# PARC-projects/video-query-algorithms

Hardware: AMD Instinct MI355X
Metric: clips/sec TSN feature-extract (higher is better)
Workload: dtype f32; 1 GPU; configs[1]: TSN BN-Inception RGB, 224x224x3, T=3, B=32/GPU (96 crops/step), crops in HBM; global_batch=32, parallelism=dp1

## Files before the change

video-query-algorithms_amd/build.py:

```python
import os
import subprocess
import sys

HERE = os.path.dirname(os.path.abspath(__file__))
ROOT = os.path.dirname(HERE)
SOURCES = ["csrc/vq_sim.hip", "csrc/vq_tsn.hip", "csrc/vq_wino.hip", "csrc/vq_boot.hip", "csrc/vq_frames.hip", "csrc/vq_comm.hip", "csrc/vq_flow.hip",
           "csrc/vq_jpeg.hip", "csrc/vq_csv.hip", "csrc/vq_rounds.hip", "csrc/vq_round_targets.hip", "csrc/vq_round_topk.hip"]
HOST_SOURCES = ["csrc/host/vq_csv.cc", "csrc/host/vq_jpeg_host.cc", "csrc/host/vq_corners.cc", "csrc/host/vq_block_pool.cc", "csrc/host/vq_tsn_plan.cc", "csrc/host/vq_flow_host.cc", "csrc/host/vq_csv_read.cc"]
HEADERS = ["csrc/vq_common.h", "csrc/vq_tsn_kernels.h", "csrc/host/vq_host.h", "csrc/host/vq_jpeg_host.h", "csrc/host/vq_corners.h", "csrc/host/vq_block_pool.h", "csrc/host/vq_tsn_plan.h", "csrc/host/vq_flow_host.h", "../include/vq_amd.h", "../include/vq_amd_rows.h", "../include/vq_amd_csv.h", "../include/vq_amd_rounds.h", "../include/vq_amd_round_views.h", "../include/vq_amd_round_fit.h", "../include/vq_amd_round_targets.h", "../include/vq_amd_round_topk.h", "../include/vq_amd_round_grid.h", "../include/vq_amd_round_update.h", "../include/vq_amd_round_shard.h",
           "csrc/vq_db.h", "csrc/vq_tile_index.h", "csrc/vq_gauss_jordan.h", "csrc/vq_select.h", "csrc/vq_score.h", "csrc/vq_decimal.h", "csrc/vq_pow5_table.h", "csrc/host/vq_csv_read.h"]
OUT = os.path.join(HERE, "libvqamd.so")
FLAGS = ["-O3", "-std=c++17", "--offload-arch=gfx950", "-fPIC", "-ffp-contract=off", "-mllvm", "-amdgpu-mfma-vgpr-form=1", "-Wall", "-Wno-unused-result",
         "-I" + os.path.join(ROOT, "include"), "-I" + os.path.join(HERE, "csrc")]
FLAGS += os.environ.get("VQ_EXTRA_HIPCC_FLAGS", "").split()


def _stale():
    if not os.path.exists(OUT):
        return True
    t = os.path.getmtime(OUT)
    return any(os.path.getmtime(os.path.join(HERE, p)) > t for p in SOURCES + HOST_SOURCES + HEADERS + ["build.py"])


def build(force=False, verbose=True):
    if not force and not _stale():
        return OUT
    hipcc = os.environ.get("HIPCC", "/opt/rocm/bin/hipcc")
    objs = []
    procs = []
    os.makedirs(os.path.join(HERE, "build"), exist_ok=True)
    for src in SOURCES:
        obj = os.path.join(HERE, "build", os.path.basename(src) + ".o")
        objs.append(obj)
        cmd = [hipcc, "-c"] + FLAGS + [os.path.join(HERE, src), "-o", obj]
        if verbose:
            print(" ".join(cmd), flush=True)
        procs.append(subprocess.Popen(cmd))
    host_flags = ["-O3", "-std=c++17", "-fPIC", "-Wall", "-I" + os.path.join(ROOT, "include"), "-I" + os.path.join(HERE, "csrc"),
                  "-I" + os.path.join(HERE, "csrc", "host")]
    for src in HOST_SOURCES:
        obj = os.path.join(HERE, "build", os.path.basename(src) + ".o")
        objs.append(obj)
        cmd = [os.environ.get("CXX", "g++"), "-c"] + host_flags + [os.path.join(HERE, src), "-o", obj]
        if verbose:
            print(" ".join(cmd), flush=True)
        procs.append(subprocess.Popen(cmd))
    for p in procs:
        if p.wait() != 0:
            raise RuntimeError("compilation failed")
    cmd = [hipcc, "-shared", "--offload-arch=gfx950", "-fPIC"] + objs + ["-o", OUT]
    if verbose:
        print(" ".join(cmd), flush=True)
    subprocess.check_call(cmd + ["-ldl", "-lpthread"])
    return OUT


if __name__ == "__main__":
    build(force="--force" in sys.argv)
```

video-query-algorithms_amd/csrc/vq_tsn.hip:

```cpp
#include <algorithm>
#include <cmath>
#include <cstring>
#include <map>
#include <set>
#include <tuple>
#include <type_traits>
#include <vector>

#include "vq_common.h"
#include "vq_tsn_kernels.h"
#include "host/vq_block_pool.h"

using namespace vq;

typedef float floatx16 __attribute__((ext_vector_type(16)));
typedef float floatx4 __attribute__((ext_vector_type(4)));
typedef unsigned uintx4 __attribute__((__vector_size__(4 * sizeof(unsigned))));

__global__ void preprocess_kernel(const uint8_t* __restrict__ src, float* __restrict__ dst, int64_t nchunk, int C, int Cpad,
                                  const float* __restrict__ mean) {
    const int64_t i = (int64_t)blockIdx.x * blockDim.x + threadIdx.x;
    if (i >= nchunk) return;
    const int cpp = Cpad >> 2;
    const int64_t p = i / cpp;
// ... 684 lines not shown
    _Pragma("unroll") for (int i = 0; i < TM; ++i)                                                                  \
        fa[SET][i] = *reinterpret_cast<const floatx4*>(a_frag + 32 * i * pitch + (G) * 8);
#define VQ_PG_MFMA(SET, BSET, Q)                                                                                    \
    _Pragma("unroll") for (int s_ = 0; s_ < 4; ++s_)                                                                \
        _Pragma("unroll") for (int i = 0; i < TM; ++i)                                                              \
            _Pragma("unroll") for (int j = 0; j < TN; ++j)                                                          \
                acc[i][j] = __builtin_amdgcn_mfma_f32_32x32x2f32(fa[SET][i][s_], fbs[BSET][Q][j][s_], acc[i][j], 0, 0, 0);
#define VQ_PG_SLAB(S, BSET)                                                                                         \
    {                                                                                                               \
        const bool more = (S) + 1 < ns;                                                                             \
        if (more) {                                                                                                 \
            VQ_PG_FETCH_B((BSET) ^ 1, (S) + 1)                                                                      \
            VQ_PG_TAPS((S) + 1)                                              \
        }                                                                                                           \
        VQ_PG_FETCH_A(0, (S) * GS)                                                                                  \
        __builtin_amdgcn_sched_barrier(0);                                                                          \
        _Pragma("unroll") for (int q = 0; q < GS; ++q) {                                                            \
            if (q + 1 < GS) VQ_PG_FETCH_A((q + 1) & 1, (S) * GS + q + 1)                                            \
            __builtin_amdgcn_sched_barrier(0);                                                                      \
            VQ_PG_MFMA(q & 1, BSET, q)                                                                              \
            __builtin_amdgcn_sched_barrier(0);                                                                      \
        }                                                                                                           \
        if (more) {                                                                                                 \
            VQ_PG_POOL((S) + 1)                                                                                     \
            __syncthreads();                                  \
        }                                                                                                           \
    }

    const int ns = K / SLAB;
    VQ_PG_FETCH_B(0, 0)
    VQ_PG_TAPS(0)
    VQ_PG_POOL(0)
    __syncthreads();
    int s = 0;
    for (; s + 1 < ns; s += 2) {
        VQ_PG_SLAB(s, 0)
        VQ_PG_SLAB(s + 1, 1)
    }
    if (s < ns) VQ_PG_SLAB(s, 0)
#undef VQ_PG_SLAB
#undef VQ_PG_TAPS
#undef VQ_PG_POOL
#undef VQ_PG_FETCH_A
#undef VQ_PG_FETCH_B
#undef VQ_PG_MFMA
    VQ_EPILOGUE()
}

template <bool IS_MAX>
__global__ __launch_bounds__(256) void pool_kernel(PoolArgs a) {
    const int64_t i = (int64_t)blockIdx.x * blockDim.x + threadIdx.x;
    if (i < a.total) pool_one<IS_MAX>(a, i);
}

__global__ void gavgpool_kernel(const float* __restrict__ in, float* __restrict__ out, int n, int HW, int Cs_in, int coff_in,
                                int C, int Cs_out, int coff_out) {
    const int i = blockIdx.x * blockDim.x + threadIdx.x;
    if (i >= n * C) return;
    const int c = i % C, img = i / C;
    const float* p = in + (size_t)img * HW * Cs_in + coff_in + c;
    float acc = 0.f;
    for (int q = 0; q < HW; ++q) acc += p[(size_t)q * Cs_in];
    out[(size_t)img * Cs_out + coff_out + c] = acc / (float)HW;
}

constexpr int FC_ROWS = 4;
__global__ __launch_bounds__(64) void inner_product_kernel(const float* __restrict__ x, int x_stride, const float* __restrict__ W,
                                                           const float* __restrict__ bias, float* __restrict__ y, int y_stride, int M,
                                                           int K, int N) {
    const int lane = threadIdx.x;
    const int m0 = blockIdx.x * FC_ROWS, n0 = blockIdx.y * FC_COLS;
    const float* xr[FC_ROWS];
    const float* wr[FC_COLS];
#pragma unroll
    for (int r = 0; r < FC_ROWS; ++r) xr[r] = x + (size_t)min(m0 + r, M - 1) * x_stride;
#pragma unroll
    for (int c = 0; c < FC_COLS; ++c) wr[c] = W + (size_t)min(n0 + c, N - 1) * K;
    float acc[FC_ROWS][FC_COLS];
#pragma unroll
    for (int r = 0; r < FC_ROWS; ++r)
#pragma unroll
        for (int c = 0; c < FC_COLS; ++c) acc[r][c] = 0.f;
    for (int k = 4 * lane; k < K; k += 256) {
        floatx4 xv[FC_ROWS], wv[FC_COLS];
#pragma unroll
        for (int r = 0; r < FC_ROWS; ++r) xv[r] = *reinterpret_cast<const floatx4*>(xr[r] + k);
#pragma unroll
        for (int c = 0; c < FC_COLS; ++c) wv[c] = *reinterpret_cast<const floatx4*>(wr[c] + k);
#pragma unroll
        for (int e = 0; e < 4; ++e)
#pragma unroll
            for (int r = 0; r < FC_ROWS; ++r)
#pragma unroll
                for (int c = 0; c < FC_COLS; ++c) acc[r][c] = __builtin_fmaf(xv[r][e], wv[c][e], acc[r][c]);
    }
    float mine = 0.f;
#pragma unroll
    for (int r = 0; r < FC_ROWS; ++r)
#pragma unroll
        for (int c = 0; c < FC_COLS; ++c) {
            float v = acc[r][c];
#pragma unroll
            for (int s = 32; s >= 1; s >>= 1) v += __shfl_xor(v, s, 64);
            if (lane == r * FC_COLS + c) mine = v;
        }
    const int m = m0 + lane / FC_COLS, n = n0 + lane % FC_COLS;
    if (lane < FC_ROWS * FC_COLS && m < M && n < N) y[(size_t)m * y_stride + n] = mine + bias[n];
}

__global__ void splitk_combine_kernel(const float* __restrict__ part, int ksplit, size_t slice_stride, int M, int Cout,
                                      const float* __restrict__ bias, int relu, float* __restrict__ out, int Cs_out) {
    const int64_t i = (int64_t)blockIdx.x * blockDim.x + threadIdx.x;
    const int c4 = Cout / 4;
    if (i >= (int64_t)M * c4) return;
    const int m = (int)(i / c4), n = (int)(i - (int64_t)m * c4) * 4;
    floatx4 v = *reinterpret_cast<const floatx4*>(part + (size_t)m * Cout + n);
    for (int q = 1; q < ksplit; ++q) v += *reinterpret_cast<const floatx4*>(part + q * slice_stride + (size_t)m * Cout + n);
    v += *reinterpret_cast<const floatx4*>(bias + n);
    if (relu) {
        v[0] = fmaxf(v[0], 0.f);
        v[1] = fmaxf(v[1], 0.f);
        v[2] = fmaxf(v[2], 0.f);
        v[3] = fmaxf(v[3], 0.f);
    }
    *reinterpret_cast<floatx4*>(out + (size_t)m * Cs_out + n) = v;
}

__global__ void gavgpool_consensus_kernel(const float* __restrict__ in, float* __restrict__ out, double* __restrict__ feat, int T,
                                          int HW, int Cs_in, int coff_in, int C, int Cs_out, int coff_out) {
    __shared__ float pooled[kMaxFusedT][64];
    const int c = blockIdx.x * 64 + threadIdx.x, t = threadIdx.y, b = blockIdx.y;
    float v = 0.f;
    if (c < C) {
        const int img = b * T + t;
        const float* p = in + (size_t)img * HW * Cs_in + coff_in + c;
        float acc = 0.f;
        int q = 0;
        for (; q + 7 <= HW; q += 7) {
            float x[7];
#pragma unroll
            for (int u = 0; u < 7; ++u) x[u] = p[(size_t)(q + u) * Cs_in];
#pragma unroll
            for (int u = 0; u < 7; ++u) acc += x[u];
        }
        for (; q < HW; ++q) acc += p[(size_t)q * Cs_in];
        v = acc / (float)HW;
        out[(size_t)img * Cs_out + coff_out + c] = v;
    }
    pooled[t][threadIdx.x] = v;
    __syncthreads();
    if (t == 0 && c < C) {
        double cons = (double)pooled[0][threadIdx.x];
        for (int s = 1; s < T; ++s) cons = cons + (double)pooled[s][threadIdx.x];
        feat[(size_t)b * C + c] = cons / (double)T;
    }
}

__global__ void consensus_kernel(const float* __restrict__ per_snippet, double* __restrict__ feat, int B, int T, int D, int Cs) {
    const int i = blockIdx.x * blockDim.x + threadIdx.x;
    if (i >= B * D) return;
    const int d = i % D, b = i / D;
    double acc = (double)per_snippet[(size_t)(b * T) * Cs + d];
    for (int t = 1; t < T; ++t) acc = acc + (double)per_snippet[(size_t)(b * T + t) * Cs + d];
    feat[i] = acc / (double)T;
}

struct Launch {
    hipStream_t stream;
    hipEvent_t ev_start, ev_stop;
    int crop0;
    int T;
    bool fused_consensus;
};

struct vq_tsn {
    std::mutex mu;
    int device = 0;
    hipStream_t stream = nullptr;
// ... 242 lines not shown
    a.coff_out = L.dst_coff;
    a.Cout = L.cout;
    a.k = L.k;
    a.kw = L.k;
    a.col_off = 4;
    a.c_step = 0;
    a.stride = L.stride;
    a.pad = L.pad;
    a.M = n_crops * td.h * td.w;
    a.Kp = (L.k * L.k * L.cin + KPAD - 1) / KPAD * KPAD;
    a.relu = L.relu;
    a.pool_k = L.pre_pool_k;
    a.pool_s = L.pre_pool_stride;
    a.ksplit = 1;
    a.k_per = 0;
    a.seg_stride = 0;
    a.tiles_m = a.tiles_n = 0;
    a.in_bytes = (unsigned)((size_t)n_crops * ts.h * ts.w * ts.c * sizeof(float));
    a.w_bytes = (unsigned)((size_t)L.cout * a.Kp * sizeof(float));
}

static int launch_conv_layer(const vq_tsn* net, const Launch& ln, int li, int n_crops, int tile_idx) {
    ConvArgs a;
    fill_conv_args(net, ln, li, n_crops, a);
    const vq_layer_desc& L = net->plan.layers[li];
    const bool stem_rows = L.src == 0 && net->plan.input.s2d_pad >= 0 && net->plan.input.s2d_order == 1;
    if (stem_rows) {
        a.k = a.kw = 1;
        a.Cin = 4 * L.k * L.cin;
        a.col_off = net->plan.tensors[L.src].w * net->plan.tensors[L.src].c;
        a.c_step = 4;
        a.Kp = stem_rows_kp(net->plan.input.c);
        a.w_bytes = (unsigned)((size_t)L.cout * a.Kp * sizeof(float));
    } else if (L.pad == 0 && L.k > 1 && L.cin == net->plan.tensors[L.src].c && L.src_coff == 0) {
        a.kw = 1;
        a.Cin = L.k * L.cin;
    }
    const ConvLaunch run = conv_launch(net, li, a, stem_rows, tile_idx);
    const ConvTile& t = kTiles[tile_idx];
    if (!run) return fail(VQ_E_INVALID, "layer %d: no kernel for tile %dx%dx%d pipe=%d", li, t.bm, t.bn, t.bk, t.pipe);
    if (net->plan.ksplit[li] == 1) return run(ln, a);
    a.ksplit = net->plan.ksplit[li];
    a.k_per = a.Kp / a.ksplit;
    a.seg_stride = (L.cout + 31) / 32;
    a.bias = net->zero_bias;
    a.out_row0 = (int)cdiv((int64_t)ln.crop0 * (int64_t)net->plan.split_crop_floats, (int64_t)L.cout);
    Launch slices = ln, combine = ln;
    slices.ev_stop = nullptr;
    combine.ev_start = nullptr;
    const int rc = run(slices, a);
    if (rc != VQ_OK) return rc;
    const vq_tensor_desc& td = net->plan.tensors[L.dst];
    float* out = net->slots[L.dst] + (size_t)ln.crop0 * td.h * td.w * td.c + L.dst_coff;
    const int64_t work = (int64_t)a.M * (L.cout / 4);
    VQ_LAUNCH(splitk_combine_kernel, (unsigned)cdiv(work, 256), 256, 0, combine.stream, combine.ev_start, combine.ev_stop,
              net->split_scratch + (size_t)a.out_row0 * L.cout, a.ksplit, net->split_slice_floats, a.M, L.cout, net->blob + L.b_off, L.relu, out, td.c);
    VQ_CHECK_LAUNCH();
    return VQ_OK;
}

static void fill_wino_job(const vq_tsn* net, const Launch& ln, int li, int n_crops, WinoJob& a, int variant) {
    const vq_layer_desc& L = net->plan.layers[li];
    const vq_tensor_desc& ts = net->plan.tensors[L.src];
    const vq_tensor_desc& td = net->plan.tensors[L.dst];
    memset(&a, 0, sizeof a);
    a.in = net->slots[L.src] + (size_t)ln.crop0 * ts.h * ts.w * ts.c;
    a.u = net->blob + L.w_off;
    a.bias = net->blob + L.b_off;
    a.out = net->slots[L.dst] + (size_t)ln.crop0 * td.h * td.w * td.c;
    a.H = ts.h;
    a.W = ts.w;
    a.Cs_in = ts.c;
    a.coff_in = L.src_coff;
    a.Cin = L.cin;
    a.Cs_out = td.c;
    a.coff_out = L.dst_coff;
    a.Cout = L.cout;
    a.th = (ts.h + 1) / 2;
    a.tw = (ts.w + 1) / 2;
    a.P = n_crops * a.th * a.tw;
    a.relu = L.relu;
    a.t16 = L.op == VQ_OP_CONV_WINOGRAD16 && variant >= 2;
    if (a.t16) a.u += (size_t)16 * L.cout * L.cin;
    a.in_bytes = (unsigned)((size_t)n_crops * ts.h * ts.w * ts.c * sizeof(float));
    a.out_bytes = (unsigned)((size_t)n_crops * td.h * td.w * td.c * sizeof(float));
    a.u_bytes = (unsigned)((size_t)16 * L.cout * L.cin * sizeof(float));
}

static void fill_pool_args(const vq_tsn* net, const Launch& ln, int li, int n_crops, PoolArgs& a) {
    const vq_layer_desc& L = net->plan.layers[li];
    const vq_tensor_desc& ts = net->plan.tensors[L.src];
    const vq_tensor_desc& td = net->plan.tensors[L.dst];
    memset(&a, 0, sizeof a);
    a.in = net->slots[L.src] + (size_t)ln.crop0 * ts.h * ts.w * ts.c;
    a.out = net->slots[L.dst] + (size_t)ln.crop0 * td.h * td.w * td.c;
    a.H = ts.h;
    a.W = ts.w;
    a.Cs_in = ts.c;
    a.coff_in = L.src_coff;
    a.C = L.cin;
    a.Ho = td.h;
    a.Wo = td.w;
    a.Cs_out = td.c;
    a.coff_out = L.dst_coff;
    a.k = L.k;
    a.stride = L.stride;
    a.pad = L.pad;
    a.is_max = L.op == VQ_OP_MAXPOOL;
    a.total = (int64_t)n_crops * td.h * td.w * (L.cin / 4);
    a.bias = (L.op == VQ_OP_AVGPOOL && L.has_bias) ? net->blob + L.b_off : nullptr;
    a.relu = (L.op == VQ_OP_AVGPOOL) ? L.relu : 0;
}

static int launch_wino_layers(const vq_tsn* net, const Launch& ln, const std::vector<int>& members, int n_crops, int variant) {
    WinoGroup g;
    memset(&g, 0, sizeof g);
    for (int li : members) {
        if (is_wino(net->plan.layers[li].op)) {
            VQ_REQUIRE(g.n_jobs < kWinoMaxJobs, "a Winograd launch carries at most %d convolutions", kWinoMaxJobs);
            fill_wino_job(net, ln, li, n_crops, g.job[g.n_jobs++], variant);
        } else {
            VQ_REQUIRE(g.n_pools < kWinoMaxPools, "a Winograd launch carries at most %d pooling layers", kWinoMaxPools);
            fill_pool_args(net, ln, li, n_crops, g.pool[g.n_pools++]);
        }
    }
    bool both = true;
    for (int li : members)
        if (net->plan.layers[li].op == VQ_OP_CONV_WINOGRAD) both = false;
    if (variant >= 2 && !both) {
        variant -= 2;
        for (int q = 0; q < g.n_jobs; ++q) VQ_REQUIRE(!g.job[q].t16, "internal: mixed Winograd layouts in one launch");
    }
    return launch_wino_group(g, variant, ln.stream, ln.ev_start, ln.ev_stop);
}

static int run_layer(const vq_tsn* net, const Launch& ln, int li, int n_crops, int tune_key);

static int run_item(const vq_tsn* net, const Launch& whole, const LaunchItem& it, int n_crops, int tune_key) {
    for (int done = 0; done < n_crops;) {
        const int n = std::min(n_crops - done, it.max_crops);
        Launch ln = whole;
        ln.crop0 = whole.crop0 + done;
        if (done != 0) ln.ev_start = nullptr;
        if (done + n != n_crops) ln.ev_stop = nullptr;
        int rc;
        if (it.kind == 1) {
            auto tn = net->tuned.find(tune_key);
            rc = launch_wino_layers(net, ln, it.layers, n, tn != net->tuned.end() ? tn->second[it.layers[0]] : 0);
        } else {
            rc = run_layer(net, ln, it.layers[0], n, tune_key);
        }
        if (rc != VQ_OK) return rc;
        done += n;
    }
    return VQ_OK;
}

constexpr int kPairedKey = 1 << 24;
static inline int tile_key(int n_crops, bool paired) { return n_crops + (paired ? kPairedKey : 0); }

struct EventSet {
    std::vector<hipEvent_t> ev;
    ~EventSet() {
        for (hipEvent_t e : ev)
// ... 74 lines not shown
        int win = seen.empty() ? 0 : seen[0].second;
        for (size_t k = 0; k < std::min<size_t>(3, seen.size()) && seen.size() > 1; ++k) {
            for (int m : it.layers) pick[m] = seen[k].second;
            float ms = 0.f;
            const int rc = timed(it, 5, &ms);
            if (rc != VQ_OK) return rc;
            if (ms < best) {
                best = ms;
                win = seen[k].second;
            }
        }
        for (int m : it.layers) pick[m] = win;
    }
    return VQ_OK;
}

static int ensure_tuned(vq_tsn* net, int n_crops, bool paired) {
    const int key = tile_key(n_crops, paired);
    if (net->forced_tile >= 0 || net->tuned.find(key) != net->tuned.end()) return VQ_OK;
    for (const bool p : {paired, !paired}) {
        std::vector<int> sizes;
        for (const auto& kv : net->tuned)
            if ((kv.first >= kPairedKey) == p && !net->tuned_borrowed.count(kv.first)) sizes.push_back(kv.first - (p ? kPairedKey : 0));
        if (const int nearest = nearest_size(sizes, n_crops)) {
            net->tuned[key] = net->tuned[tile_key(nearest, p)];
            net->tuned_borrowed.insert(key);
            return VQ_OK;
        }
    }
    if (!net->autotune) return VQ_OK;
    return autotune(net, n_crops, paired);
}

static int run_layer(const vq_tsn* net, const Launch& ln, int li, int n_crops, int tune_key) {
    const vq_layer_desc& L = net->plan.layers[li];
    const vq_tensor_desc& ts = net->plan.tensors[L.src];
    const vq_tensor_desc& td = net->plan.tensors[L.dst];
    if (L.op == VQ_OP_CONV) {
        int t = net->forced_tile;
        if (t < 0) {
            auto it = net->tuned.find(tune_key);
            t = it != net->tuned.end() ? it->second[li] : heuristic_tile(net, li, n_crops);
        }
        return launch_conv_layer(net, ln, li, n_crops, t);
    }
    if (is_wino(L.op)) {
        auto it = net->tuned.find(tune_key);
        return launch_wino_layers(net, ln, std::vector<int>{li}, n_crops, it != net->tuned.end() ? it->second[li] : 0);
    }
    if (L.op == VQ_OP_MAXPOOL || L.op == VQ_OP_AVGPOOL) {
        PoolArgs a;
        fill_pool_args(net, ln, li, n_crops, a);
        const int64_t blocks = (a.total + 255) / 256;
        if (L.op == VQ_OP_MAXPOOL)
            VQ_LAUNCH(pool_kernel<true>, (unsigned)blocks, 256, 0, ln.stream, ln.ev_start, ln.ev_stop, a);
        else
            VQ_LAUNCH(pool_kernel<false>, (unsigned)blocks, 256, 0, ln.stream, ln.ev_start, ln.ev_stop, a);
        VQ_CHECK_LAUNCH();
        return VQ_OK;
    }
    if (L.op == VQ_OP_GLOBAL_AVGPOOL) {
        const float* gin = net->slots[L.src] + (size_t)ln.crop0 * ts.h * ts.w * ts.c;
        float* gout = net->slots[L.dst] + (size_t)ln.crop0 * td.c;
        const int T = ln.T;
        if (li == net->plan.consensus_layer && ln.fused_consensus) {
            const int B = n_crops / T;
            VQ_LAUNCH(gavgpool_consensus_kernel, dim3(cdiv(L.cin, 64), B), dim3(64, T), 0, ln.stream, ln.ev_start, ln.ev_stop, gin, gout,
                      net->feat_dev + (size_t)(ln.crop0 / T) * net->plan.D, T, ts.h * ts.w, ts.c, L.src_coff, L.cin, td.c, L.dst_coff);
        } else {
            VQ_LAUNCH(gavgpool_kernel, cdiv((int64_t)n_crops * L.cin, 256), 256, 0, ln.stream, ln.ev_start, ln.ev_stop, gin, gout, n_crops,
                      ts.h * ts.w, ts.c, L.src_coff, L.cin, td.c, L.dst_coff);
        }
        VQ_CHECK_LAUNCH();
        return VQ_OK;
    }
    if (L.op == VQ_OP_INNER_PRODUCT) {
        const float* xin = net->slots[L.src] + (size_t)ln.crop0 * ts.c + L.src_coff;
        float* yout = net->slots[L.dst] + (size_t)ln.crop0 * td.c + L.dst_coff;
        VQ_LAUNCH(inner_product_kernel, dim3(cdiv(n_crops, FC_ROWS), cdiv(L.cout, FC_COLS)), 64, 0, ln.stream, ln.ev_start, ln.ev_stop, xin, ts.c,
                  net->blob + L.w_off, net->blob + L.b_off, yout, td.c, n_crops, L.cin, L.cout);
        VQ_CHECK_LAUNCH();
        return VQ_OK;
    }
    return fail(VQ_E_INVALID, "layer %d: unknown op %d", li, L.op);
}

extern "C" {

int vq_tsn_create(const vq_tensor_desc* tensors, int32_t n_tensors, const vq_layer_desc* layers, int32_t n_layers,
                  const vq_conv_segment* segments, int32_t n_segments, const float* blob_host, int64_t blob_floats,
                  const vq_input_desc* input, int32_t feature_slot, int32_t max_crops, int32_t device, vq_tsn** out) {
    VQ_REQUIRE(out, "out is NULL");
    *out = nullptr;
    TsnPlan plan;
    const int vrc = validate_plan(tensors, n_tensors, layers, n_layers, segments, n_segments, blob_host, blob_floats, input, feature_slot, max_crops, &plan);
    if (vrc != VQ_OK) return vrc;
    const int in_channels = input->c;
    int ndev = 0;
    VQ_HIP(hipGetDeviceCount(&ndev));
    VQ_REQUIRE(device >= 0 && device < ndev, "device %d out of range (%d visible)", device, ndev);
    DeviceGuard g(device);
    auto* net = new vq_tsn;
    net->device = device;
    net->max_crops = max_crops;
    net->in_channels = in_channels;
    net->plan = std::move(plan);
    net->feature_slot = feature_slot;
// ... 499 lines not shown
```

video-query-algorithms_amd/csrc/vq_tsn_kernels.h:

```cpp
#pragma once
#include <hip/hip_runtime.h>
#include <hip/hip_ext.h>

#include "host/vq_tsn_plan.h"

namespace vq {

__device__ __forceinline__ int xcd_remap(int bid, int nwg) {
    const int q = nwg >> 3, r = nwg & 7, xcd = bid & 7, idx = bid >> 3;
    return (xcd < r ? xcd * (q + 1) : r * (q + 1) + (xcd - r) * q) + idx;
}

__device__ __forceinline__ unsigned magic_div(unsigned x, unsigned m) { return m ? __umulhi(x, m) : x; }

struct FullDiv {
    unsigned m, sh1, sh2;
};
__device__ __forceinline__ unsigned full_div(unsigned x, const FullDiv& d) {
    const unsigned t = __umulhi(d.m, x);
    return (t + ((x - t) >> d.sh1)) >> d.sh2;
}
static inline FullDiv full_div_for(unsigned d) {
    unsigned l = 0;
    while ((1ull << l) < d) ++l;
    FullDiv f;
    f.m = (unsigned)(((1ull << 32) * ((1ull << l) - d)) / d + 1);
    f.sh1 = l < 1 ? l : 1;
    f.sh2 = l > 1 ? l - 1 : 0;
    return f;
}
constexpr int kRecipShift = 22;
__device__ __forceinline__ unsigned umul24(unsigned x, unsigned y_uniform) {
    unsigned r;
    asm("v_mul_u32_u24 %0, %2, %1" : "=v"(r) : "v"(x), "s"(y_uniform));
    return r;
}
__device__ __forceinline__ int imul24(int x, int y_uniform) {
    int r;
    asm("v_mul_i32_i24 %0, %2, %1" : "=v"(r) : "v"(x), "s"(y_uniform));
    return r;
}
static inline unsigned recip22(unsigned d) { return (1u << kRecipShift) / d + 1u; }
static inline bool recip22_ok(unsigned d, unsigned xmax) {
    return d >= 1 && (unsigned long long)xmax * d < (1ull << kRecipShift) && (unsigned long long)xmax * recip22(d) < (1ull << 32);
}

struct PoolArgs {
    const float* in;
    float* out;
    int H, W, Cs_in, coff_in, C;
    int Ho, Wo, Cs_out, coff_out;
    int k, stride, pad;
    int is_max;
    int64_t total;
    const float* bias;
    int relu;
    int unit0, n_units;
};
constexpr int kPoolPerWG = 1024;

template <bool IS_MAX>
__device__ __forceinline__ void pool_one(const PoolArgs& a, int64_t i) {
    const int c4n = a.C >> 2;
    const int c4 = (int)(i % c4n);
    int64_t pix = i / c4n;
    const int pw = (int)(pix % a.Wo);
    pix /= a.Wo;
    const int ph = (int)(pix % a.Ho);
    const int64_t n = pix / a.Ho;
    int hs = ph * a.stride - a.pad, ws = pw * a.stride - a.pad;
    int he = min(hs + a.k, a.H + a.pad), we = min(ws + a.k, a.W + a.pad);
    const float pool_size = (float)((he - hs) * (we - ws));
    hs = max(hs, 0);
    ws = max(ws, 0);
    he = min(he, a.H);
    we = min(we, a.W);
    const float* base = a.in + (size_t)n * a.H * a.W * a.Cs_in + a.coff_in + c4 * 4;
    float4 acc = IS_MAX ? make_float4(-INFINITY, -INFINITY, -INFINITY, -INFINITY) : make_float4(0.f, 0.f, 0.f, 0.f);
    for (int h = hs; h < he; ++h)
        for (int w = ws; w < we; ++w) {
            const float4 v = *reinterpret_cast<const float4*>(base + ((size_t)h * a.W + w) * a.Cs_in);
            if (IS_MAX) {
                acc.x = fmaxf(acc.x, v.x);
                acc.y = fmaxf(acc.y, v.y);
                acc.z = fmaxf(acc.z, v.z);
                acc.w = fmaxf(acc.w, v.w);
            } else {
                acc.x += v.x;
                acc.y += v.y;
                acc.z += v.z;
                acc.w += v.w;
            }
        }
    if (!IS_MAX) {
        acc.x /= pool_size;
        acc.y /= pool_size;
        acc.z /= pool_size;
        acc.w /= pool_size;
        if (a.bias) {
            const float4 b = *reinterpret_cast<const float4*>(a.bias + c4 * 4);
            acc.x += b.x;
            acc.y += b.y;
            acc.z += b.z;
            acc.w += b.w;
        }
        if (a.relu) {
            acc.x = fmaxf(acc.x, 0.f);
            acc.y = fmaxf(acc.y, 0.f);
            acc.z = fmaxf(acc.z, 0.f);
            acc.w = fmaxf(acc.w, 0.f);
        }
    }
// ... 47 lines not shown
```

video-query-algorithms_amd/csrc/vq_wino.hip:

```cpp
#include "vq_common.h"
#include "vq_tsn_kernels.h"

using namespace vq;

typedef float floatx16 __attribute__((ext_vector_type(16)));
typedef float floatx4 __attribute__((ext_vector_type(4)));
typedef float floatx2 __attribute__((ext_vector_type(2)));
typedef unsigned uintx4 __attribute__((__vector_size__(4 * sizeof(unsigned))));

namespace {

__device__ __forceinline__ floatx2 pk_add2(floatx2 x, floatx2 y) {
    floatx2 r;
    asm("v_pk_add_f32 %0, %1, %2" : "=v"(r) : "v"(x), "v"(y));
    return r;
}
__device__ __forceinline__ floatx2 pk_sub2(floatx2 x, floatx2 y) {
    floatx2 r;
    asm("v_pk_add_f32 %0, %1, %2 neg_lo:[0,1] neg_hi:[0,1]" : "=v"(r) : "v"(x), "v"(y));
    return r;
}
__device__ __forceinline__ floatx4 pk_add(floatx4 x, floatx4 y) {
    const floatx2 lo = pk_add2(x.xy, y.xy), hi = pk_add2(x.zw, y.zw);
    return (floatx4){lo.x, lo.y, hi.x, hi.y};
// ... 391 lines not shown
    for (int nb = 0; nb < NB; ++nb) {
#pragma unroll
        for (int bb = 0; bb < 2; ++bb) {
            const int b = 2 * nb + bb;
            floatx4 t0, t1;
#pragma unroll
            for (int h2 = 0; h2 < 2; ++h2) {
                const floatx2 m0 = {acc[0][b][2 * h2], acc[0][b][2 * h2 + 1]}, m1 = {acc[1][b][2 * h2], acc[1][b][2 * h2 + 1]};
                const floatx2 m2 = {acc[2][b][2 * h2], acc[2][b][2 * h2 + 1]}, m3 = {acc[3][b][2 * h2], acc[3][b][2 * h2 + 1]};
                const floatx2 s0 = pk_add2(pk_add2(m0, m1), m2), s1 = pk_sub2(pk_sub2(m1, m2), m3);
                t0[2 * h2] = s0.x;
                t0[2 * h2 + 1] = s0.y;
                t1[2 * h2] = s1.x;
                t1[2 * h2 + 1] = s1.y;
            }
            *reinterpret_cast<floatx4*>(ep_w + 16 * bb) = t0;
            *reinterpret_cast<floatx4*>(ep_w + BP16 * EP_ROW + 16 * bb) = t1;
        }
        __syncthreads();
        {
            const floatx4 v0 = *reinterpret_cast<const floatx4*>(ep_r + (0 * 2 + bsel) * BP16 * EP_ROW);
            const floatx4 v1 = *reinterpret_cast<const floatx4*>(ep_r + (1 * 2 + bsel) * BP16 * EP_ROW);
            const floatx4 v2 = *reinterpret_cast<const floatx4*>(ep_r + (2 * 2 + bsel) * BP16 * EP_ROW);
            const floatx4 v3 = *reinterpret_cast<const floatx4*>(ep_r + (3 * 2 + bsel) * BP16 * EP_ROW);
            floatx4 y0 = pk_add(pk_add(v0, v1), v2);
            floatx4 y1 = pk_sub(pk_sub(v1, v2), v3);
            if (a.relu) {
#pragma unroll
                for (int r = 0; r < 4; ++r) {
                    y0[r] = relu1(y0[r]);
                    y1[r] = relu1(y1[r]);
                }
            }
            const bool blk_ok = n0 + 32 * nb < a.Cout;
            __builtin_amdgcn_raw_buffer_store_b128(__builtin_bit_cast(uintx4, y0), out_rsrc, blk_ok ? ooff[0] : 0xFFFFFFFFu, nb * (32 * 4), 0);
            __builtin_amdgcn_raw_buffer_store_b128(__builtin_bit_cast(uintx4, y1), out_rsrc, blk_ok ? ooff[1] : 0xFFFFFFFFu, nb * (32 * 4), 0);
        }
        if (nb + 1 < NB) __syncthreads();
    }
}

template <int NB, int TB>
__global__ __launch_bounds__(256) __attribute__((amdgpu_waves_per_eu(NB == 1 ? 4 : 2, NB == 1 ? 4 : 2)))
void wino_f2x2_3x3_kernel(WinoGroup g) {
    extern __shared__ __attribute__((aligned(16))) char smem_raw[];
    float* hs = reinterpret_cast<float*>(smem_raw);
    const int b = blockIdx.x;
    if (b >= g.pool_unit0) {
        int q = 0;
        if (g.n_pools > 1 && b >= g.pool[1].unit0) q = 1;
        const PoolArgs& pa = g.pool[q];
        const int unit = b - pa.unit0;
        if (unit >= pa.n_units) return;
#pragma unroll
        for (int r = 0; r < kPoolPerWG / 256; ++r) {
            const int64_t i = (int64_t)unit * kPoolPerWG + r * 256 + threadIdx.x;
            if (i < pa.total) {
                if (pa.is_max)
                    pool_one<true>(pa, i);
                else
                    pool_one<false>(pa, i);
            }
        }
        return;
    }
    int j = 0;
#pragma unroll
    for (int q = 1; q < kWinoMaxJobs; ++q)
        if (q < g.n_jobs && b >= g.job[q].unit0) j = q;
    const WinoJob& a = g.job[j];
    const int unit = b - a.unit0;
    if (unit >= a.n_units) return;
    if constexpr (TB == 16)
        wino16_unit<NB>(a, unit, hs);
    else
        wino_unit<NB>(a, unit, hs);
}

unsigned magic_u32(unsigned d) { return d == 1 ? 0u : (unsigned)(0x100000000ull / d) + 1u; }

template <int NB, int TB>
int launch_t(WinoGroup& g, hipStream_t stream, hipEvent_t ev_start, hipEvent_t ev_stop) {
    int units = 0;
    for (int q = 0; q < g.n_jobs; ++q) {
        WinoJob& a = g.job[q];
        a.tiles_n = cdiv(a.Cout, 32 * NB);
        const long long n = (long long)cdiv(a.P, TB) * a.tiles_n;
        VQ_REQUIRE(n > 0 && n < (1 << 24), "Winograd job %d: %lld workgroups", q, n);
        a.unit0 = units;
        a.n_units = (int)n;
        units += ((int)n + 7) & ~7;
        const unsigned tpi = (unsigned)(a.th * a.tw);
        VQ_REQUIRE((unsigned long long)n * a.tiles_n < 0x100000000ull && (unsigned long long)(a.P + BP) * tpi < 0x100000000ull &&
                       recip22_ok((unsigned)a.tw, (unsigned)a.tw + BP) && recip22_ok((unsigned)a.th, (unsigned)a.th + BP + 2),
                   "Winograd job %d: shape outside the reciprocal-division range", q);
        VQ_REQUIRE((unsigned long long)cdiv(a.P, (int)tpi) * a.H * a.W < (1ull << 23) && a.Cs_in < (1 << 23) && a.Cs_out < (1 << 23),
                   "Winograd job %d: more than 2^23 pixels in a slot (split the batch)", q);
        a.m_tiles_n = magic_u32((unsigned)a.tiles_n);
        a.m_tpi = magic_u32(tpi);
        a.m_tw = magic_u32((unsigned)a.tw);
        a.s_tw = recip22((unsigned)a.tw);
        a.s_th = recip22((unsigned)a.th);
    }
    g.pool_unit0 = units;
    for (int q = 0; q < g.n_pools; ++q) {
        PoolArgs& pa = g.pool[q];
// ... 38 lines not shown
```

Before: 12580 clips/s.

## Add specialized 3x3 pooling path with buffer loads and 2D split-K combine grid

Adds a fast pooling path for 3x3 stride-1 pad-1 and stride-2 pad-0 pools. It uses reciprocal-based 24-bit index math, raw buffer loads with out-of-range masking for padding, packed adds, max3, and software-pipelined tap fetches. The path is used both as a standalone kernel and inside the fused Winograd group. The split-K combine kernel is also reshaped to a 2D grid with 32-bit offsets, guarded by a new size check. Both changes aim to cut integer division cost and 64-bit addressing overhead in memory-bound stages, at the cost of more code and tight range preconditions.

```diff
diff --git a/video-query-algorithms_amd/build.py b/video-query-algorithms_amd/build.py
--- a/video-query-algorithms_amd/build.py
+++ b/video-query-algorithms_amd/build.py
@@ -7,7 +7,7 @@
 SOURCES = ["csrc/vq_sim.hip", "csrc/vq_tsn.hip", "csrc/vq_wino.hip", "csrc/vq_boot.hip", "csrc/vq_frames.hip", "csrc/vq_comm.hip", "csrc/vq_flow.hip",
            "csrc/vq_jpeg.hip", "csrc/vq_csv.hip", "csrc/vq_rounds.hip", "csrc/vq_round_targets.hip", "csrc/vq_round_topk.hip"]
 HOST_SOURCES = ["csrc/host/vq_csv.cc", "csrc/host/vq_jpeg_host.cc", "csrc/host/vq_corners.cc", "csrc/host/vq_block_pool.cc", "csrc/host/vq_tsn_plan.cc", "csrc/host/vq_flow_host.cc", "csrc/host/vq_csv_read.cc"]
-HEADERS = ["csrc/vq_common.h", "csrc/vq_tsn_kernels.h", "csrc/host/vq_host.h", "csrc/host/vq_jpeg_host.h", "csrc/host/vq_corners.h", "csrc/host/vq_block_pool.h", "csrc/host/vq_tsn_plan.h", "csrc/host/vq_flow_host.h", "../include/vq_amd.h", "../include/vq_amd_rows.h", "../include/vq_amd_csv.h", "../include/vq_amd_rounds.h", "../include/vq_amd_round_views.h", "../include/vq_amd_round_fit.h", "../include/vq_amd_round_targets.h", "../include/vq_amd_round_topk.h", "../include/vq_amd_round_grid.h", "../include/vq_amd_round_update.h", "../include/vq_amd_round_shard.h",
+HEADERS = ["csrc/vq_common.h", "csrc/vq_tsn_kernels.h", "csrc/vq_div9.h","csrc/host/vq_host.h", "csrc/host/vq_jpeg_host.h", "csrc/host/vq_corners.h", "csrc/host/vq_block_pool.h", "csrc/host/vq_tsn_plan.h", "csrc/host/vq_flow_host.h", "../include/vq_amd.h", "../include/vq_amd_rows.h", "../include/vq_amd_csv.h", "../include/vq_amd_rounds.h", "../include/vq_amd_round_views.h", "../include/vq_amd_round_fit.h", "../include/vq_amd_round_targets.h", "../include/vq_amd_round_topk.h", "../include/vq_amd_round_grid.h", "../include/vq_amd_round_update.h", "../include/vq_amd_round_shard.h",
            "csrc/vq_db.h", "csrc/vq_tile_index.h", "csrc/vq_gauss_jordan.h", "csrc/vq_select.h", "csrc/vq_score.h", "csrc/vq_decimal.h", "csrc/vq_pow5_table.h", "csrc/host/vq_csv_read.h"]
 OUT = os.path.join(HERE, "libvqamd.so")
 FLAGS = ["-O3", "-std=c++17", "--offload-arch=gfx950", "-fPIC", "-ffp-contract=off", "-mllvm", "-amdgpu-mfma-vgpr-form=1", "-Wall", "-Wno-unused-result",
diff --git a/video-query-algorithms_amd/csrc/vq_div9.h b/video-query-algorithms_amd/csrc/vq_div9.h
--- /dev/null
+++ b/video-query-algorithms_amd/csrc/vq_div9.h
@@ -0,0 +1,19 @@
+#pragma once
+
+#if defined(__HIPCC__)
+#define VQ_DIV9_FN __host__ __device__ __forceinline__
+#else
+#define VQ_DIV9_FN static inline
+#endif
+
+namespace vq {
+
+VQ_DIV9_FN float div9(float a) {
+    const float z = 1.0f / 9.0f;
+    const float q = a * z;
+    const float r = __builtin_fmaf(-9.0f, q, a);
+    const float c = __builtin_fmaf(r, z, q);
+    return (q == 0.0f || __builtin_isinf(q)) ? q : c;
+}
+
+}
diff --git a/video-query-algorithms_amd/csrc/vq_tsn.hip b/video-query-algorithms_amd/csrc/vq_tsn.hip
--- a/video-query-algorithms_amd/csrc/vq_tsn.hip
+++ b/video-query-algorithms_amd/csrc/vq_tsn.hip
@@ -760,6 +760,7 @@
     const int64_t i = (int64_t)blockIdx.x * blockDim.x + threadIdx.x;
     if (i < a.total) pool_one<IS_MAX>(a, i);
 }
+__global__ __launch_bounds__(256) void pool_fast_kernel(PoolArgs a) { pool_unit_any(a, blockIdx.x); }
 
 __global__ void gavgpool_kernel(const float* __restrict__ in, float* __restrict__ out, int n, int HW, int Cs_in, int coff_in,
                                 int C, int Cs_out, int coff_out) {
@@ -816,14 +817,16 @@
     if (lane < FC_ROWS * FC_COLS && m < M && n < N) y[(size_t)m * y_stride + n] = mine + bias[n];
 }
 
-__global__ void splitk_combine_kernel(const float* __restrict__ part, int ksplit, size_t slice_stride, int M, int Cout,
-                                      const float* __restrict__ bias, int relu, float* __restrict__ out, int Cs_out) {
-    const int64_t i = (int64_t)blockIdx.x * blockDim.x + threadIdx.x;
-    const int c4 = Cout / 4;
-    if (i >= (int64_t)M * c4) return;
-    const int m = (int)(i / c4), n = (int)(i - (int64_t)m * c4) * 4;
-    floatx4 v = *reinterpret_cast<const floatx4*>(part + (size_t)m * Cout + n);
-    for (int q = 1; q < ksplit; ++q) v += *reinterpret_cast<const floatx4*>(part + q * slice_stride + (size_t)m * Cout + n);
+__global__ __launch_bounds__(256) void splitk_combine_kernel(const float* __restrict__ part, int ksplit, size_t slice_stride, int M, int Cout,
+                                                             const float* __restrict__ bias, int relu, float* __restrict__ out, int Cs_out) {
+    const unsigned m = blockIdx.x * 4u + (threadIdx.x >> 6), n = (blockIdx.y * 64u + (threadIdx.x & 63u)) * 4u;
+    if (m >= (unsigned)M || n >= (unsigned)Cout) return;
+    const unsigned at = m * (unsigned)Cout + n;
+    floatx4 v = *reinterpret_cast<const floatx4*>(part + at);
+    for (int q = 1; q < ksplit; ++q) {
+        part += slice_stride;
+        v += *reinterpret_cast<const floatx4*>(part + at);
+    }
     v += *reinterpret_cast<const floatx4*>(bias + n);
     if (relu) {
         v[0] = fmaxf(v[0], 0.f);
@@ -831,7 +834,7 @@
         v[2] = fmaxf(v[2], 0.f);
         v[3] = fmaxf(v[3], 0.f);
     }
-    *reinterpret_cast<floatx4*>(out + (size_t)m * Cs_out + n) = v;
+    *reinterpret_cast<floatx4*>(out + (m * (unsigned)Cs_out + n)) = v;
 }
 
 __global__ void gavgpool_consensus_kernel(const float* __restrict__ in, float* __restrict__ out, double* __restrict__ feat, int T,
@@ -1180,8 +1183,8 @@
     if (rc != VQ_OK) return rc;
     const vq_tensor_desc& td = net->plan.tensors[L.dst];
     float* out = net->slots[L.dst] + (size_t)ln.crop0 * td.h * td.w * td.c + L.dst_coff;
-    const int64_t work = (int64_t)a.M * (L.cout / 4);
-    VQ_LAUNCH(splitk_combine_kernel, (unsigned)cdiv(work, 256), 256, 0, combine.stream, combine.ev_start, combine.ev_stop,
+    VQ_REQUIRE((int64_t)a.M * L.cout < (1ll << 31) && (int64_t)a.M * td.c < (1ll << 31), "layer %d: K-split combine pass beyond 32-bit offsets (split the batch)", li);
+    VQ_LAUNCH(splitk_combine_kernel, dim3((unsigned)cdiv(a.M, 4), (unsigned)cdiv(L.cout / 4, 64)), 256, 0, combine.stream, combine.ev_start, combine.ev_stop,
               net->split_scratch + (size_t)a.out_row0 * L.cout, a.ksplit, net->split_slice_floats, a.M, L.cout, net->blob + L.b_off, L.relu, out, td.c);
     VQ_CHECK_LAUNCH();
     return VQ_OK;
@@ -1238,6 +1241,10 @@
     a.total = (int64_t)n_crops * td.h * td.w * (L.cin / 4);
     a.bias = (L.op == VQ_OP_AVGPOOL && L.has_bias) ? net->blob + L.b_off : nullptr;
     a.relu = (L.op == VQ_OP_AVGPOOL) ? L.relu : 0;
+    const size_t in_bytes = (size_t)n_crops * ts.h * ts.w * ts.c * sizeof(float), out_bytes = (size_t)n_crops * td.h * td.w * td.c * sizeof(float);
+    a.in_bytes = in_bytes <= 0x7FFFFFF0u ? (unsigned)in_bytes : 0u;
+    a.out_bytes = out_bytes <= 0x7FFFFFF0u ? (unsigned)out_bytes : 0u;
+    pool_plan(a, n_crops);
 }
 
 static int launch_wino_layers(const vq_tsn* net, const Launch& ln, const std::vector<int>& members, int n_crops, int variant) {
@@ -1418,7 +1425,9 @@
         PoolArgs a;
         fill_pool_args(net, ln, li, n_crops, a);
         const int64_t blocks = (a.total + 255) / 256;
-        if (L.op == VQ_OP_MAXPOOL)
+        if (a.mode)
+            VQ_LAUNCH(pool_fast_kernel, (unsigned)((a.total + kPoolPerWG - 1) / kPoolPerWG), 256, 0, ln.stream, ln.ev_start, ln.ev_stop, a);
+        else if (L.op == VQ_OP_MAXPOOL)
             VQ_LAUNCH(pool_kernel<true>, (unsigned)blocks, 256, 0, ln.stream, ln.ev_start, ln.ev_stop, a);
         else
             VQ_LAUNCH(pool_kernel<false>, (unsigned)blocks, 256, 0, ln.stream, ln.ev_start, ln.ev_stop, a);
diff --git a/video-query-algorithms_amd/csrc/vq_tsn_kernels.h b/video-query-algorithms_amd/csrc/vq_tsn_kernels.h
--- a/video-query-algorithms_amd/csrc/vq_tsn_kernels.h
+++ b/video-query-algorithms_amd/csrc/vq_tsn_kernels.h
@@ -3,6 +3,7 @@
 #include <hip/hip_ext.h>
 
 #include "host/vq_tsn_plan.h"
+#include "vq_div9.h"
 
 namespace vq {
 
@@ -56,8 +57,152 @@
     const float* bias;
     int relu;
     int unit0, n_units;
+    int mode;
+    unsigned in_bytes, out_bytes;
+    FullDiv d_c4n, d_wo, d_ho;
+    unsigned s_c4n, s_wo, s_ho;
 };
 constexpr int kPoolPerWG = 1024;
+constexpr int kPool311 = 1, kPool320 = 2;
+
+static inline void pool_plan(PoolArgs& a, int n_crops) {
+    a.mode = 0;
+    const bool w311 = a.k == 3 && a.stride == 1 && a.pad == 1 && a.Ho == a.H && a.Wo == a.W;
+    const bool w320 = a.k == 3 && a.stride == 2 && a.pad == 0 && a.Ho >= 1 && a.Wo >= 1 && 2 * (a.Ho - 1) < a.H && 2 * (a.Wo - 1) < a.W;
+    if (!w311 && !w320) return;
+    const unsigned c4n = (unsigned)(a.C >> 2);
+    if (a.C < 4 || a.C % 4 || a.Cs_in % 4 || a.coff_in % 4 || a.Cs_out % 4 || a.coff_out % 4) return;
+    if (a.in_bytes > 0x7FFFFFF0u || a.out_bytes > 0x7FFFFFF0u || a.in_bytes == 0 || a.out_bytes == 0) return;
+    if (a.total <= 0 || a.total + kPoolPerWG >= (1ll << 31)) return;
+    if ((long long)n_crops * a.H * a.W + a.W + 2 >= (1 << 23) || (long long)n_crops * a.Ho * a.Wo + kPoolPerWG >= (1 << 23) ||
+        a.Cs_in >= (1 << 21) || a.Cs_out >= (1 << 21))
+        return;
+    if (!recip22_ok(c4n, c4n + kPoolPerWG) || !recip22_ok((unsigned)a.Wo, (unsigned)a.Wo + kPoolPerWG) ||
+        !recip22_ok((unsigned)a.Ho, (unsigned)a.Ho + kPoolPerWG))
+        return;
+    a.d_c4n = full_div_for(c4n);
+    a.d_wo = full_div_for((unsigned)a.Wo);
+    a.d_ho = full_div_for((unsigned)a.Ho);
+    a.s_c4n = recip22(c4n);
+    a.s_wo = recip22((unsigned)a.Wo);
+    a.s_ho = recip22((unsigned)a.Ho);
+    a.mode = w311 ? kPool311 : kPool320;
+}
+
+typedef float poolx4 __attribute__((ext_vector_type(4)));
+typedef float poolx2 __attribute__((ext_vector_type(2)));
+typedef unsigned pooluintx4 __attribute__((__vector_size__(4 * sizeof(unsigned))));
+
+__device__ __forceinline__ float max3(float x, float y, float z) {
+    float r;
+    asm("v_max3_f32 %0, %1, %2, %3" : "=v"(r) : "v"(x), "v"(y), "v"(z));
+    return r;
+}
+__device__ __forceinline__ float max0(float x) {
+    float r;
+    asm("v_max_f32 %0, 0, %1" : "=v"(r) : "v"(x));
+    return r;
+}
+__device__ __forceinline__ poolx4 pool_add(poolx4 x, poolx4 y) {
+    poolx2 lo, hi;
+    asm("v_pk_add_f32 %0, %1, %2" : "=v"(lo) : "v"(x.xy), "v"(y.xy));
+    asm("v_pk_add_f32 %0, %1, %2" : "=v"(hi) : "v"(x.zw), "v"(y.zw));
+    return (poolx4){lo.x, lo.y, hi.x, hi.y};
+}
+
+struct PoolTaps {
+    poolx4 v[9];
+    poolx4 b;
+    unsigned ooff;
+    float size;
+};
+
+template <int MODE, bool IS_MAX>
+__device__ __forceinline__ void pool_unit(const PoolArgs& a, unsigned unit) {
+    constexpr int S = MODE == kPool311 ? 1 : 2, P = MODE == kPool311 ? 1 : 0, R = kPoolPerWG / 256;
+    constexpr unsigned kRowOut = 0x80000000u, kColOut = 0x7FFFFFF0u;
+    const unsigned c4n = (unsigned)a.C >> 2, H = (unsigned)a.H, W = (unsigned)a.W, Ho = (unsigned)a.Ho, Wo = (unsigned)a.Wo;
+    const unsigned first = unit * (unsigned)kPoolPerWG;
+    const unsigned pix0 = full_div(first, a.d_c4n), c40 = first - pix0 * c4n;
+    const unsigned row0 = full_div(pix0, a.d_wo), pw0 = pix0 - row0 * Wo;
+    const unsigned n0 = full_div(row0, a.d_ho), ph0 = row0 - n0 * Ho;
+    const unsigned s_c4n = a.s_c4n, s_wo = a.s_wo, s_ho = a.s_ho;
+    const unsigned left = (unsigned)a.total - first;
+    const int px = a.Cs_in * 4, opx = a.Cs_out * 4, cin0 = a.coff_in * 4, cout0 = a.coff_out * 4;
+    const bool has_bias = !IS_MAX && a.bias != nullptr, relu = !IS_MAX && a.relu != 0;
+    const __amdgpu_buffer_rsrc_t in_rsrc = __builtin_amdgcn_make_buffer_rsrc(const_cast<float*>(a.in), 0, a.in_bytes, 0x00020000);
+    const __amdgpu_buffer_rsrc_t out_rsrc = __builtin_amdgcn_make_buffer_rsrc(a.out, 0, a.out_bytes, 0x00020000);
+    const __amdgpu_buffer_rsrc_t b_rsrc = __builtin_amdgcn_make_buffer_rsrc(const_cast<float*>(a.bias), 0, has_bias ? (unsigned)a.C * 4u : 0u, 0x00020000);
+
+    PoolTaps t[2];
+    auto request = [&](int r, PoolTaps& q) {
+        const unsigned e = (unsigned)(r * 256) + threadIdx.x;
+        const unsigned x = c40 + e, dp = umul24(x, s_c4n) >> kRecipShift, c4 = x - umul24(dp, c4n);
+        const unsigned y = pw0 + dp, dq = umul24(y, s_wo) >> kRecipShift, pw = y - umul24(dq, Wo);
+        const unsigned z = ph0 + dq, dn = umul24(z, s_ho) >> kRecipShift, ph = z - umul24(dn, Ho);
+        const int nH = imul24((int)(n0 + dn), (int)H);
+        const int hs = (int)ph * S - P, ws = (int)pw * S - P;
+        const int cb = cin0 + (int)c4 * 16;
+        unsigned ro[3], co[3];
+#pragma unroll
+        for (int d = 0; d < 3; ++d) {
+            const int h = IS_MAX ? min(max(hs + d, 0), (int)H - 1) : hs + d, w = IS_MAX ? min(max(ws + d, 0), (int)W - 1) : ws + d;
+            const unsigned rb = (unsigned)(imul24(imul24(nH + h, (int)W), px) + cb), cbyte = (unsigned)imul24(w, px);
+            ro[d] = IS_MAX || (unsigned)h < H ? rb : kRowOut;
+            co[d] = IS_MAX || (unsigned)w < W ? cbyte : kColOut;
+        }
+#pragma unroll
+        for (int dh = 0; dh < 3; ++dh)
+#pragma unroll
+            for (int dw = 0; dw < 3; ++dw)
+                q.v[dh * 3 + dw] = __builtin_bit_cast(poolx4, __builtin_amdgcn_raw_buffer_load_b128(in_rsrc, ro[dh] + co[dw], 0, 0));
+        if (has_bias) q.b = __builtin_bit_cast(poolx4, __builtin_amdgcn_raw_buffer_load_b128(b_rsrc, c4 * 16u, 0, 0));
+        const unsigned obyte = umul24(pix0 + dp, (unsigned)opx) + (unsigned)cout0 + c4 * 16u;
+        q.ooff = e < left ? obyte : 0xFFFFFFFFu;
+        if (!IS_MAX && MODE != kPool311)
+            q.size = (float)(min(hs + 3, (int)H + P) - hs) * (float)(min(ws + 3, (int)W + P) - ws);
+    };
+    auto finish = [&](const PoolTaps& q) {
+        poolx4 acc;
+        if (IS_MAX) {
+#pragma unroll
+            for (int c = 0; c < 4; ++c)
+                acc[c] = max3(max3(q.v[0][c], q.v[1][c], q.v[2][c]), max3(q.v[3][c], q.v[4][c], q.v[5][c]), max3(q.v[6][c], q.v[7][c], q.v[8][c]));
+        } else {
+            acc = pool_add((poolx4){0.f, 0.f, 0.f, 0.f}, q.v[0]);
+#pragma unroll
+            for (int k = 1; k < 9; ++k) acc = pool_add(acc, q.v[k]);
+#pragma unroll
+            for (int c = 0; c < 4; ++c) acc[c] = MODE == kPool311 ? div9(acc[c]) : acc[c] / q.size;
+            if (has_bias) acc = pool_add(acc, q.b);
+            if (relu) {
+#pragma unroll
+                for (int c = 0; c < 4; ++c) acc[c] = max0(acc[c]);
+            }
+        }
+        __builtin_amdgcn_raw_buffer_store_b128(__builtin_bit_cast(pooluintx4, acc), out_rsrc, q.ooff, 0, 0);
+    };
+    request(0, t[0]);
+#pragma unroll
+    for (int r = 0; r < R; ++r) {
+        if (r + 1 < R) request(r + 1, t[(r + 1) & 1]);
+        finish(t[r & 1]);
+    }
+}
+
+__device__ __forceinline__ void pool_unit_any(const PoolArgs& a, unsigned unit) {
+    if (a.mode == kPool311) {
+        if (a.is_max)
+            pool_unit<kPool311, true>(a, unit);
+        else
+            pool_unit<kPool311, false>(a, unit);
+    } else {
+        if (a.is_max)
+            pool_unit<kPool320, true>(a, unit);
+        else
+            pool_unit<kPool320, false>(a, unit);
+    }
+}
 
 template <bool IS_MAX>
 __device__ __forceinline__ void pool_one(const PoolArgs& a, int64_t i) {
diff --git a/video-query-algorithms_amd/csrc/vq_wino.hip b/video-query-algorithms_amd/csrc/vq_wino.hip
--- a/video-query-algorithms_amd/csrc/vq_wino.hip
+++ b/video-query-algorithms_amd/csrc/vq_wino.hip
@@ -467,6 +467,10 @@
         const PoolArgs& pa = g.pool[q];
         const int unit = b - pa.unit0;
         if (unit >= pa.n_units) return;
+        if (pa.mode) {
+            pool_unit_any(pa, (unsigned)unit);
+            return;
+        }
 #pragma unroll
         for (int r = 0; r < kPoolPerWG / 256; ++r) {
             const int64_t i = (int64_t)unit * kPoolPerWG + r * 256 + threadIdx.x;
```

Result: faster. 12960 clips/s (median of 6 runs) (+2.9%).
